# lmcinnes/pynndescent

Measured on AMD Instinct MI355X. Metric: index build: points indexed/sec (recall@10 vs brute force reported alongside), higher is better.
Workload: dtype f32

## Files before the change

pynndescent_amd/csrc/leaf_join.hip:

```cpp
#include <type_traits>

#include "common.h"
#include "metric.h"
#include "gram.h"
#include "merge.h"
#include "state.h"

#ifndef NND_LEAF_QW_OCC
#define NND_LEAF_QW_OCC 6
#endif
template <int NT, int NW, int DC, bool QW = false>
struct leaf_cfg {
    static constexpr int MP = NT * 16;
    static constexpr int TR = (NT + NW - 1) / NW;
    static constexpr int DSTRIDE = MP + 1;
    static constexpr int XS_FLOATS = MP * DC;
    static constexpr bool FULLD = NT <= 6;
    static constexpr int TPW = (NT * (NT + 1) / 2 + NW - 1) / NW;
    static constexpr int DB_FLOATS = FULLD ? MP * DSTRIDE : NW * 16 * DSTRIDE;
    static constexpr int QPASS = (MP + NW * 4 - 1) / (NW * 4);
    static constexpr bool PREFETCH = FULLD && !QW;
    static constexpr int PRE_FLOATS = PREFETCH ? MP * 16 * 2 : 0;
    static constexpr int EPI_FLOATS = DB_FLOATS + PRE_FLOATS;
    static constexpr int BIG_FLOATS = XS_FLOATS > EPI_FLOATS ? XS_FLOATS : EPI_FLOATS;
};

template <int NT, int NW, int DC, bool QW = false>
__global__ __launch_bounds__(NW * 64, (NT <= 5 && NW == 8) ? 8 : (QW && NT <= 5 && NW == 4) ? NND_LEAF_QW_OCC : 1) void k_leaf_join(const float *__restrict__ xp, int dp, const float *__restrict__ nrm,
                                                       int metric, const int32_t *__restrict__ perm,
                                                       const int32_t *__restrict__ wl_start,
                                                       const int32_t *__restrict__ wl_len, int64_t leaf0,
                                                       int64_t n_leaves, int k, int ks, uint32_t *__restrict__ knn_e,
                                                       float *__restrict__ knn_d, float *__restrict__ th,
                                                       long long *__restrict__ counters, int m_lo) {
    using C = leaf_cfg<NT, NW, DC, QW>;
    static_assert(!QW || C::FULLD, "quarter-wave merges read the whole distance block from LDS");
    __shared__ __attribute__((aligned(16))) float big[C::BIG_FLOATS];
    __shared__ int32_t ids[C::MP];
    __shared__ float nrs[C::MP];
    __shared__ uint2 qscr[QW ? NW * 4 * NND_Q16B_CAP : 1];
#ifdef NND_LEAF_PAD_LDS
    __shared__ float lds_pad[NND_LEAF_PAD_LDS];
    if (dp < 0) lds_pad[threadIdx.x] = 1.0f, counters[0] = (long long)lds_pad[(threadIdx.x + 1) & 63];
#endif

    const int tid = threadIdx.x, lane = nnd_lane(), w = tid >> 6;
    const int64_t leaf = leaf0 + blockIdx.x;
    if (leaf >= n_leaves) return;
    const int start = wl_start[leaf];
    const int m = wl_len[leaf];
    if (m < 2) return;
    if (m <= m_lo || m > C::MP) return;
    const int nt = (m + 15) >> 4;
    const int mp = nt << 4;

    for (int r = tid; r < C::MP; r += NW * 64) ids[r] = r < m ? perm[start + r] : -1;
    __syncthreads();

    constexpr int NTHR = NW * 64;
    constexpr int NLD = (C::MP * (DC / 4) + NTHR - 1) / NTHR;
    constexpr int NKL = (C::MP * 16 + NTHR - 1) / NTHR;
    constexpr bool quarter = QW;
    const bool use_pre = !quarter && C::PREFETCH && ks <= 16 && (m * ks * 2 <= C::BIG_FLOATS - C::DB_FLOATS);
    uint32_t qe[C::QPASS];
    float qd[C::QPASS];
    float *Xs = big;
    uint32_t pe[NKL];
    float pd[NKL];
    f32x4 acc[C::TR][NT];
    f32x4 acct[C::TPW];
    int tI[C::TPW], tJ[C::TPW];
    bool tOn[C::TPW];
#pragma unroll
    for (int tr = 0; tr < C::TR; tr++)
#pragma unroll
        for (int J = 0; J < NT; J++) acc[tr][J] = f32x4{0.f, 0.f, 0.f, 0.f};
#pragma unroll
    for (int q = 0; q < C::TPW; q++) {
        acct[q] = f32x4{0.f, 0.f, 0.f, 0.f};
        int t = w + q * NW, I = 0;
        while (I < nt && t >= nt - I) {
            t -= nt - I;
            I++;
        }
        tOn[q] = I < nt;
        tI[q] = I < nt ? I : 0;
        tJ[q] = I < nt ? I + t : 0;
    }

    for (int c0 = 0; c0 < dp; c0 += DC) {
        const int cw = (dp - c0) < DC ? (dp - c0) : DC;
        {
            static_assert(DC == 64, "cw is 32 or 64 (dp is a multiple of 32): chunk index by shift");
            const int nch = cw >> 2, total = mp * nch, nsh = cw == 64 ? 4 : 3;
            f32x4 rv[NLD];
#pragma unroll
            for (int q = 0; q < NLD; q++) {
                const int idx = tid + q * NTHR, idc = idx < total ? idx : 0;
                const int r = idc >> nsh, ch = idc & (nch - 1);
                const int id = ids[r];
                rv[q] = *(const f32x4 *)(xp + (int64_t)(id >= 0 ? id : 0) * dp + c0 + 4 * ch);
            }
            float my_nrm = 0.0f;
            if (c0 == 0) {
                if (!QW && tid < C::MP) {
                    const int id = ids[tid];
                    my_nrm = nrm[id >= 0 ? id : 0];
                }
                if constexpr (quarter) {
#pragma unroll
                    for (int q = 0; q < C::QPASS; q++) {
                        const int i = q * NW * 4 + (tid >> 4), j = lane & 15;
                        const bool on = i < m && j < k;
                        const int64_t v = ids[i < m ? i : 0];
                        const uint32_t ev = knn_e[v * ks + (on ? j : 0)];
                        const float dv = knn_d[v * ks + (on ? j : 0)];
                        qe[q] = on ? ev : NND_EMPTY_E;
                        qd[q] = on ? dv : INFINITY;
                    }
                }
                if (use_pre) {
#pragma unroll
                    for (int q = 0; q < NKL; q++) {
                        const int idx = tid + q * NTHR, idc = idx < m * ks ? idx : 0;
                        const int i = idc / ks, j = idc - i * ks;
                        pe[q] = knn_e[(int64_t)ids[i] * ks + j];
                        pd[q] = knn_d[(int64_t)ids[i] * ks + j];
                    }
                }
            }
            if (c0 > 0) __syncthreads();
#pragma unroll
            for (int q = 0; q < NLD; q++) {
                const int idx = tid + q * NTHR;
                if (idx < total) {
                    const int r = idx >> nsh, ch = idx & (nch - 1);
                    *(f32x4 *)&Xs[nnd_swz<DC>(r, ch)] = rv[q];
                }
            }
            if (!QW && c0 == 0 && tid < C::MP) nrs[tid] = my_nrm;
        }
        __syncthreads();
        if constexpr (C::FULLD) {
            const int lr = lane & 15, lg = lane >> 4;
            auto run = [&](auto nq_tag) {
                constexpr int NQ = decltype(nq_tag)::value;
#ifdef NND_LEAF_NOGRAM
                for (int t = 0; t < 1; t++) {
#else
                for (int t = 0; t < (cw >> 4); t++) {
#endif
                    const int c = 4 * t + lg;
                    float4 a[NQ], b[NQ];
#pragma unroll
                    for (int q = 0; q < NQ; q++) {
                        a[q] = *(const float4 *)&Xs[nnd_swz<DC>(tI[q] * 16 + lr, c)];
                        b[q] = *(const float4 *)&Xs[nnd_swz<DC>(tJ[q] * 16 + lr, c)];
                    }
#pragma unroll
                    for (int q = 0; q < NQ; q++) acct[q] = __builtin_amdgcn_mfma_f32_16x16x4f32(a[q].x, b[q].x, acct[q], 0, 0, 0);
#pragma unroll
                    for (int q = 0; q < NQ; q++) acct[q] = __builtin_amdgcn_mfma_f32_16x16x4f32(a[q].y, b[q].y, acct[q], 0, 0, 0);
#pragma unroll
                    for (int q = 0; q < NQ; q++) acct[q] = __builtin_amdgcn_mfma_f32_16x16x4f32(a[q].z, b[q].z, acct[q], 0, 0, 0);
#pragma unroll
                    for (int q = 0; q < NQ; q++) acct[q] = __builtin_amdgcn_mfma_f32_16x16x4f32(a[q].w, b[q].w, acct[q], 0, 0, 0);
                }
            };
            int nq = 0;
#pragma unroll
            for (int q = 0; q < C::TPW; q++) nq += tOn[q] ? 1 : 0;
            static_assert(C::TPW <= 4, "slot dispatch below");
            if (nq == 1) run(std::integral_constant<int, 1>{});
            else if (nq == 2) run(std::integral_constant<int, C::TPW >= 2 ? 2 : 1>{});
            else if (nq == 3) run(std::integral_constant<int, C::TPW >= 3 ? 3 : 1>{});
            else if (nq == 4) run(std::integral_constant<int, C::TPW >= 4 ? 4 : 1>{});
        } else {
#pragma unroll
            for (int tr = 0; tr < C::TR; tr++) {
                const int I = w + tr * NW;
                if (I < nt) nnd_gram_chunk<DC, NT>(Xs, I * 16, 0, cw, acc[tr], [nt](int J) { return J < nt; });
            }
        }
    }
    if constexpr (QW) {
        const int r16d = lane & 15, gd = lane >> 4;
#pragma unroll
        for (int q = 0; q < C::TPW; q++) {
            if (!tOn[q] || tI[q] != tJ[q]) continue;
#pragma unroll
            for (int r = 0; r < 4; r++)
                if (4 * gd + r == r16d) nrs[tI[q] * 16 + r16d] = acct[q][r];
        }
    }
    __syncthreads();

    const int r16 = lane & 15, g = lane >> 4;
    int accepted = 0;
    if constexpr (C::FULLD) {
        float *Dm = big;
#pragma unroll
        for (int q = 0; q < C::TPW; q++) {
            if (!tOn[q]) continue;
            const int I = tI[q], J = tJ[q];
            const int j = J * 16 + r16;
            const float nj = nrs[j];
#pragma unroll
            for (int r = 0; r < 4; r++) {
                const int il = I * 16 + 4 * g + r;
                const float dv = nnd_gram_to_dist<NND_CODES_ANY>(metric, acct[q][r], nrs[il], nj);
                Dm[il * C::DSTRIDE + j] = dv;
                if (I != J) Dm[j * C::DSTRIDE + il] = dv;
            }
        }
        uint32_t *pre_e = (uint32_t *)(big + C::DB_FLOATS);
        float *pre_d = big + C::DB_FLOATS + m * ks;
        if (use_pre) {
#pragma unroll
            for (int q = 0; q < NKL; q++) {
                const int idx = tid + q * NTHR;
                if (idx < m * ks) {
                    pre_e[idx] = pe[q];
                    pre_d[idx] = pd[q];
                }
            }
        }
        __syncthreads();
        if constexpr (quarter) {
#pragma unroll
            for (int q = 0; q < C::QPASS; q++) {
                if (q * NW * 4 + w * 4 >= m) break;
                const int i = q * NW * 4 + (tid >> 4);
                const bool on = i < m;
                const float *Drow = Dm + (on ? i : 0) * C::DSTRIDE;
                const int64_t v = ids[on ? i : 0];
#ifdef NND_LEAF_NOMERGE
                if (qe[q] == 12345u && qd[q] == 3.0f && Drow[lane] == 7.0f) accepted++;
                if (false)
#endif
#ifdef NND_LEAF_OLD_MERGE
                accepted += nnd_merge_rows_q16<NT>(on, knn_e + v * ks, knn_d + v * ks, th + v, qe[q], qd[q], k, m,
                                                   [&](int c, uint32_t &id, float &dc) {
                                                       id = (uint32_t)ids[c];
                                                       dc = Drow[c];
                                                       return c != i;
                                                   });
#else
                accepted += nnd_merge_rows_q16b<NT>(on, knn_e + v * ks, knn_d + v * ks, th + v, qe[q], qd[q], k, m,
                                                    [&](int c, uint32_t &id, float &dc) {
                                                        id = (uint32_t)ids[c];
                                                        dc = Drow[c];
                                                        return c != i;
                                                    }, qscr + w * 4 * NND_Q16B_CAP);
#endif
            }
        } else
        for (int i = w; i < m; i += NW) {
            const float *Drow = Dm + i * C::DSTRIDE;
            const int64_t v = ids[i];
            uint32_t e0 = NND_EMPTY_E;
            float d0 = INFINITY;
            if (lane < k) {
                if (use_pre) {
                    e0 = pre_e[i * ks + lane];
                    d0 = pre_d[i * ks + lane];
                } else {
                    e0 = knn_e[v * ks + lane];
                    d0 = knn_d[v * ks + lane];
                }
            }
            auto cf = [&](int c, uint32_t &id, float &dc) {
                id = (uint32_t)ids[c];
                dc = Drow[c];
                return c != i;
            };
#ifdef NND_LEAF_NOMERGE
            if (e0 == 12345u && d0 == 3.0f && Drow[lane] == 7.0f) accepted++;
            if (false)
#endif
            if (C::MP > 64 && m <= 64)
                accepted += nnd_merge_row_regs<1>(knn_e + v * ks, knn_d + v * ks, th + v, e0, d0, k, m, cf);
            else
                accepted += nnd_merge_row_regs<(C::MP + 63) / 64>(knn_e + v * ks, knn_d + v * ks, th + v, e0, d0, k, m, cf);
        }
    } else {
        float *Dw = big + w * 16 * C::DSTRIDE;
#pragma unroll
        for (int tr = 0; tr < C::TR; tr++) {
            const int I = w + tr * NW;
            if (I >= nt) continue;
#pragma unroll
            for (int J = 0; J < NT; J++) {
                if (J < nt) {
                    const int j = J * 16 + r16;
                    const float nj = nrs[j];
#pragma unroll
                    for (int r = 0; r < 4; r++) {
                        const int il = 4 * g + r;
                        Dw[il * C::DSTRIDE + j] = nnd_gram_to_dist<NND_CODES_ANY>(metric, acc[tr][J][r], nrs[I * 16 + il], nj);
                    }
                }
            }
            nnd_wave_lds_sync();
            const int lk = lane < k ? lane : 0;
            uint32_t e_nx = knn_e[(int64_t)ids[I * 16] * ks + lk];
            float d_nx = knn_d[(int64_t)ids[I * 16] * ks + lk];
            for (int il = 0; il < 16; il++) {
                const int i = I * 16 + il;
                if (i >= m) break;
                const float *Drow = Dw + il * C::DSTRIDE;
                const int64_t v = ids[i];
                const uint32_t e0 = lane < k ? e_nx : NND_EMPTY_E;
                const float d0 = lane < k ? d_nx : INFINITY;
                if (il + 1 < 16 && i + 1 < m) {
                    const int64_t vn = ids[i + 1];
                    e_nx = knn_e[vn * ks + lk];
                    d_nx = knn_d[vn * ks + lk];
                }
                accepted += nnd_merge_row_regs<(C::MP + 63) / 64>(knn_e + v * ks, knn_d + v * ks, th + v, e0, d0, k, m,
                                                                 [&](int c, uint32_t &id, float &dc) {
                                                                     id = (uint32_t)ids[c];
                                                                     dc = Drow[c];
                                                                     return c != i;
                                                                 });
            }
            nnd_wave_lds_sync();
        }
    }
    __syncthreads();
    int *wacc = (int *)nrs;
    if (lane == 0) wacc[w] = accepted;
    __syncthreads();
    if (tid == 0) {
        long long a = 0;
        for (int i = 0; i < NW; i++) a += wacc[i];
        nnd_count(counters, CNT_ACCEPT, a);
        nnd_count(counters, CNT_PAIRS, (long long)m * (m - 1) / 2);
        nnd_count(counters, CNT_ROWS, m);
        nnd_count(counters, CNT_MFMA, (long long)(C::FULLD ? nt * (nt + 1) / 2 : nt * nt) * (dp >> 2));
    }
}

template <int NT, int NW = 8, bool WIDE = false>
__global__ __launch_bounds__(NW * 64, 2) void k_leaf_join_rb(const float *__restrict__ xp, int dp, const float *__restrict__ nrm, int metric,
                                                         const int32_t *__restrict__ perm, const int32_t *__restrict__ wl_start,
                                                         const int32_t *__restrict__ wl_len, int64_t leaf0, int64_t n_leaves, int k, int ks,
                                                         uint32_t *__restrict__ knn_e, float *__restrict__ knn_d, float *__restrict__ th,
                                                         long long *__restrict__ counters) {
    constexpr int DC = 64, MP = NT * 16, RB = NW * 8, TRB = RB / 16, DSTRIDE = MP + 1;
    constexpr int TPW = (TRB * NT + NW - 1) / NW;
    constexpr int NLD = (MP * (DC / 4) + NW * 64 - 1) / (NW * 64);
    constexpr int BIG = MP * DC > RB * DSTRIDE ? MP * DC : RB * DSTRIDE;
    __shared__ __attribute__((aligned(16))) float big[BIG];
    __shared__ int32_t ids[MP];
    __shared__ float nrs[MP];
    __shared__ uint64_t wide_scr[WIDE ? NW : 1][WIDE ? NND_WIDE_SCRATCH_WORDS : 1];
    const int tid = threadIdx.x, lane = nnd_lane(), w = tid >> 6;
    const int64_t leaf = leaf0 + blockIdx.x;
    if (leaf >= n_leaves) return;
    const int start = wl_start[leaf], m = wl_len[leaf];
    const int r0 = blockIdx.y * RB;
    if (m < 2 || r0 >= m) return;
    const int nt = (m + 15) >> 4, mp = nt << 4;
    for (int r = tid; r < MP; r += NW * 64) {
        const int id = r < m ? perm[start + r] : -1;
        ids[r] = id;
        nrs[r] = nrm[id >= 0 ? id : 0];
    }
    __syncthreads();
    f32x4 acc[TPW];
    int tI[TPW], tJ[TPW];
    bool tOn[TPW];
#pragma unroll
    for (int q = 0; q < TPW; q++) {
        acc[q] = f32x4{0.f, 0.f, 0.f, 0.f};
        const int t = w + q * NW;
        const int I = t / nt, J = t - I * nt;
        tOn[q] = t < TRB * nt && (r0 >> 4) + I < nt;
        tI[q] = tOn[q] ? (r0 >> 4) + I : 0;
        tJ[q] = tOn[q] ? J : 0;
    }
    float *Xs = big;
    const int r16 = lane & 15, g = lane >> 4;
    for (int c0 = 0; c0 < dp; c0 += DC) {
        const int cw = (dp - c0) < DC ? (dp - c0) : DC;
        const int nch = cw >> 2, total = mp * nch, nsh = cw == 64 ? 4 : 3;
        f32x4 rv[NLD];
#pragma unroll
        for (int q = 0; q < NLD; q++) {
            const int idx = tid + q * NW * 64, idc = idx < total ? idx : 0;
            const int r = idc >> nsh, ch = idc & (nch - 1);
            const int id = ids[r];
            rv[q] = *(const f32x4 *)(xp + (int64_t)(id >= 0 ? id : 0) * dp + c0 + 4 * ch);
        }
        if (c0 > 0) __syncthreads();
#pragma unroll
        for (int q = 0; q < NLD; q++) {
            const int idx = tid + q * NW * 64;
            if (idx < total) {
                const int r = idx >> nsh, ch = idx & (nch - 1);
                *(f32x4 *)&Xs[nnd_swz<DC>(r, ch)] = rv[q];
            }
        }
        __syncthreads();
        for (int t = 0; t < (cw >> 4); t++) {
            const int c = 4 * t + g;
            float4 a[TPW], b[TPW];
#pragma unroll
            for (int q = 0; q < TPW; q++) {
                a[q] = *(const float4 *)&Xs[nnd_swz<DC>(tI[q] * 16 + r16, c)];
                b[q] = *(const float4 *)&Xs[nnd_swz<DC>(tJ[q] * 16 + r16, c)];
            }
#pragma unroll
            for (int q = 0; q < TPW; q++) acc[q] = __builtin_amdgcn_mfma_f32_16x16x4f32(a[q].x, b[q].x, acc[q], 0, 0, 0);
#pragma unroll
            for (int q = 0; q < TPW; q++) acc[q] = __builtin_amdgcn_mfma_f32_16x16x4f32(a[q].y, b[q].y, acc[q], 0, 0, 0);
#pragma unroll
            for (int q = 0; q < TPW; q++) acc[q] = __builtin_amdgcn_mfma_f32_16x16x4f32(a[q].z, b[q].z, acc[q], 0, 0, 0);
#pragma unroll
            for (int q = 0; q < TPW; q++) acc[q] = __builtin_amdgcn_mfma_f32_16x16x4f32(a[q].w, b[q].w, acc[q], 0, 0, 0);
        }
    }
// ... 163 lines not shown
        for (int r = 0; r < 4; r++) acc[q][r] = nnd_gram_to_dist<NND_CODES_ANY>(metric, acc[q][r], nrs[tI[q] * 16 + 4 * g + r], nj);
    }
    float *Dm = big;
    int accepted = 0;
    const int j32 = lane & 31, h = lane >> 5;
    for (int p0 = 0; p0 < m; p0 += RB) {
        uint32_t pe[SPW];
        float pd[SPW];
#pragma unroll
        for (int st = 0; st < SPW; st++) {
            const int i = p0 + w * (2 * SPW) + 2 * st + h;
            const bool on = i < m && j32 < k;
            const int64_t v = ids[i < m ? i : 0];
            const uint32_t ev = knn_e[v * ks + (on ? j32 : 0)];
            const float dv = knn_d[v * ks + (on ? j32 : 0)];
            pe[st] = on ? ev : NND_EMPTY_E;
            pd[st] = on ? dv : INFINITY;
        }
        __syncthreads();
#pragma unroll
        for (int q = 0; q < TPW; q++) {
            if (!tOn[q]) continue;
            const int I = tI[q], J = tJ[q];
            if (I * 16 >= p0 && I * 16 < p0 + RB) {
#pragma unroll
                for (int r = 0; r < 4; r++) Dm[(I * 16 + 4 * g + r - p0) * DSTRIDE + J * 16 + r16] = acc[q][r];
            }
            if (I != J && J * 16 >= p0 && J * 16 < p0 + RB) {
#pragma unroll
                for (int r = 0; r < 4; r++) Dm[(J * 16 + r16 - p0) * DSTRIDE + I * 16 + 4 * g + r] = acc[q][r];
            }
        }
        __syncthreads();
#pragma unroll
        for (int st = 0; st < SPW; st++) {
            if (p0 + w * (2 * SPW) + 2 * st >= m) break;
            const int i = p0 + w * (2 * SPW) + 2 * st + h;
            const bool on = i < m;
            const float *Drow = Dm + (on ? i - p0 : 0) * DSTRIDE;
            const int64_t v = ids[on ? i : 0];
            accepted += nnd_merge_rows_q32b(on, knn_e + v * ks, knn_d + v * ks, th + v, pe[st], pd[st], k, m,
                                            [&](int c, uint32_t &id, float &dc) {
                                                id = (uint32_t)ids[c];
                                                dc = Drow[c];
                                                return c != i;
                                            }, qscr + w * 2 * NND_Q32B_CAP);
        }
    }
    __syncthreads();
    int *wacc = (int *)nrs;
    if (lane == 0) wacc[w] = accepted;
    __syncthreads();
    if (tid == 0) {
        long long a = 0;
        for (int q = 0; q < NW; q++) a += wacc[q];
        nnd_count(counters, CNT_ACCEPT, a);
        nnd_count(counters, CNT_PAIRS, (long long)m * (m - 1) / 2);
        nnd_count(counters, CNT_ROWS, m);
        nnd_count(counters, CNT_MFMA, (long long)(nt * (nt + 1) / 2) * (dp >> 2));
    }
}

static constexpr int LEAF_MAX = 256;

static int run_leaf_rounds(nnd_ctx *ctx, const int32_t *perm, const int32_t *d_ws, const int32_t *d_wl,
                           const std::vector<int64_t> &tb, int maxlen) {
    if (nnd_zero_counters(ctx)) return 1;
    const int T = (int)tb.size() - 1;
    for (int t = 0; t < T; t++) {
        int64_t cnt = tb[t + 1] - tb[t];
        if (cnt <= 0) continue;
        dim3 grid((unsigned)cnt);
#define LEAF_ARGS ctx->xp, ctx->dp, ctx->nrm, ctx->p.metric, perm, d_ws, d_wl, tb[t], tb[t + 1], ctx->k, ctx->ks, \
                  ctx->knn_e, ctx->knn_d, ctx->th, ctx->counters
        const bool qw = ctx->k <= 16;
        if (ctx->k > NND_MAX_K) {
            if (maxlen <= 128)
                hipLaunchKernelGGL((k_leaf_join_rb<8, 8, true>), dim3((unsigned)cnt, 2), dim3(512), 0, ctx->stream, LEAF_ARGS);
            else if (maxlen <= 160)
                hipLaunchKernelGGL((k_leaf_join_rb<10, 8, true>), dim3((unsigned)cnt, 3), dim3(512), 0, ctx->stream, LEAF_ARGS);
            else
                hipLaunchKernelGGL((k_leaf_join_rb<16, 8, true>), dim3((unsigned)cnt, 4), dim3(512), 0, ctx->stream, LEAF_ARGS);
        }
#ifndef NND_LEAF_OLD_K32
        else if (!qw && ctx->k <= 32 && maxlen <= 160) {
            hipLaunchKernelGGL((k_leaf_join_sym<6, 8>), grid, dim3(512), 0, ctx->stream, LEAF_ARGS, 0);
            if (maxlen > 96) hipLaunchKernelGGL((k_leaf_join_sym<10, 8>), grid, dim3(512), 0, ctx->stream, LEAF_ARGS, 96);
        }
#endif
        else if (maxlen <= 64 && qw)
            hipLaunchKernelGGL((k_leaf_join<4, 8, 64, true>), grid, dim3(512), 0, ctx->stream, LEAF_ARGS, 0);
        else if (maxlen <= 64)
            hipLaunchKernelGGL((k_leaf_join<4, 8, 64>), grid, dim3(512), 0, ctx->stream, LEAF_ARGS, 0);
        else if (maxlen <= 80 && qw) {
#ifdef NND_LEAF_ONE_CLASS
            hipLaunchKernelGGL((k_leaf_join<5, 8, 64, true>), grid, dim3(512), 0, ctx->stream, LEAF_ARGS, 0);
#else
            hipLaunchKernelGGL((k_leaf_join<4, 4, 64, true>), grid, dim3(256), 0, ctx->stream, LEAF_ARGS, 0);
#ifdef NND_LEAF_EMPTY_L
            hipLaunchKernelGGL((k_leaf_join<5, 8, 64, true>), grid, dim3(512), 0, ctx->stream, LEAF_ARGS, 1000);
#elif defined(NND_LEAF_L_NW4)
            hipLaunchKernelGGL((k_leaf_join<5, 4, 64, true>), grid, dim3(256), 0, ctx->stream, LEAF_ARGS, 64);
#else
            hipLaunchKernelGGL((k_leaf_join<5, 8, 64, true>), grid, dim3(512), 0, ctx->stream, LEAF_ARGS, 64);
#endif
#endif
        }
        else if (maxlen <= 80)
            hipLaunchKernelGGL((k_leaf_join<5, 8, 64>), grid, dim3(512), 0, ctx->stream, LEAF_ARGS, 0);
        else if (maxlen <= 96 && qw)
            hipLaunchKernelGGL((k_leaf_join<6, 8, 64, true>), grid, dim3(512), 0, ctx->stream, LEAF_ARGS, 0);
        else if (maxlen <= 96)
            hipLaunchKernelGGL((k_leaf_join<6, 8, 64>), grid, dim3(512), 0, ctx->stream, LEAF_ARGS, 0);
        else if (maxlen <= 128)
            hipLaunchKernelGGL((k_leaf_join_rb<8, 8>), dim3((unsigned)cnt, 2), dim3(512), 0, ctx->stream, LEAF_ARGS);
        else if (maxlen <= 160)
            hipLaunchKernelGGL((k_leaf_join_rb<10, 8>), dim3((unsigned)cnt, 3), dim3(512), 0, ctx->stream, LEAF_ARGS);
        else
            hipLaunchKernelGGL((k_leaf_join_rb<16, 8>), dim3((unsigned)cnt, 4), dim3(512), 0, ctx->stream, LEAF_ARGS);
#undef LEAF_ARGS
    }
    NND_HIP_CHECK(hipGetLastError());
    if (nnd_read_counters(ctx)) return 1;
    ctx->stats.leaf_pairs = ctx->h_counters[CNT_PAIRS];
    ctx->stats.leaf_rows = ctx->h_counters[CNT_ROWS];
    ctx->stats.leaf_mfma = ctx->h_counters[CNT_MFMA];
    return 0;
}

int nnd_launch_leaf_init(nnd_ctx *ctx) {
    if (!ctx->forest_built || ctx->n_leaves == 0) return 0;
    const int T = (int)ctx->tree_leaf_begin.size() - 1;
    const int32_t *d_ws = ctx->leaf_start, *d_wl = ctx->leaf_len;
    std::vector<int64_t> tb(ctx->tree_leaf_begin.begin(), ctx->tree_leaf_begin.end());
    int maxlen = ctx->max_leaf;
    if (ctx->max_leaf > LEAF_MAX) {
        if (nnd_fetch_leaf_tables(ctx)) return 1;
        const std::vector<int32_t> &hs = ctx->h_leaf_start, &hl = ctx->h_leaf_len;
        std::vector<int32_t> ws, wl;
        ws.reserve(ctx->n_leaves);
        wl.reserve(ctx->n_leaves);
        maxlen = 0;
        for (int t = 0; t < T; t++) {
            tb[t] = (int64_t)ws.size();
            for (int64_t i = ctx->tree_leaf_begin[t]; i < ctx->tree_leaf_begin[t + 1]; i++) {
                int32_t a = hs[i], len = hl[i];
                while (len > 0) {
                    int32_t piece = len > LEAF_MAX ? LEAF_MAX : len;
                    ws.push_back(a);
                    wl.push_back(piece);
                    if (piece > maxlen) maxlen = piece;
                    a += piece;
                    len -= piece;
                }
            }
        }
        tb[T] = (int64_t)ws.size();
        const int64_t nw = (int64_t)ws.size();
        if (nw == 0) return 0;
        if (!ctx->mem.grow2(&ctx->wl_start, &ctx->wl_len, &ctx->wl_cap, nw, nw + nw / 4)) { ctx->set_error("out of device memory for the leaf work list"); return 1; }
        NND_HIP_CHECK(hipMemcpyAsync(ctx->wl_start, ws.data(), sizeof(int32_t) * nw, hipMemcpyHostToDevice, ctx->stream));
        NND_HIP_CHECK(hipMemcpyAsync(ctx->wl_len, wl.data(), sizeof(int32_t) * nw, hipMemcpyHostToDevice, ctx->stream));
        NND_HIP_CHECK(hipStreamSynchronize(ctx->stream));
        d_ws = ctx->wl_start;
        d_wl = ctx->wl_len;
    }
    return run_leaf_rounds(ctx, ctx->perm[ctx->cur], d_ws, d_wl, tb, maxlen);
}


int nnd_launch_leaf_init_array(nnd_ctx *ctx, const int32_t *leaf_host, int64_t n_leaves, int32_t max_leaf_size) {
    if (n_leaves <= 0 || max_leaf_size <= 0) return 0;
    const int64_t n = ctx->n;
    std::vector<int32_t> seen((size_t)n, 0);
    struct piece { int64_t off; int32_t len; int32_t round; };
    std::vector<piece> pieces;
    pieces.reserve((size_t)n_leaves);
    int n_rounds = 0, maxlen = 0;
    for (int64_t l = 0; l < n_leaves; l++) {
        const int32_t *row = leaf_host + l * max_leaf_size;
        int32_t len = 0;
        while (len < max_leaf_size && row[len] >= 0) {
            if ((int64_t)row[len] >= n) { ctx->set_error("nnd_init_from_leaf_array: leaf %lld holds point %d but n = %lld", (long long)l, row[len], (long long)n); return 1; }
            len++;
        }
        if (len < 2) continue;
        int32_t r = 0;
        for (int32_t i = 0; i < len; i++) r = seen[row[i]] > r ? seen[row[i]] : r;
        for (int32_t i = 0; i < len; i++) {
// ... 39 lines not shown
```

pynndescent_amd/csrc/merge.h:

```cpp
#pragma once
#include "common.h"

#define NND_MAX_K 64

__device__ __forceinline__ uint64_t nnd_readlane_u64(uint64_t v, int src_lane) {
    uint32_t lo = (uint32_t)__builtin_amdgcn_readlane((int)(uint32_t)v, src_lane);
    uint32_t hi = (uint32_t)__builtin_amdgcn_readlane((int)(uint32_t)(v >> 32), src_lane);
    return ((uint64_t)hi << 32) | lo;
}

template <int NCHUNK, typename CandFn>
__device__ __forceinline__ int nnd_merge_row_regs(uint32_t *__restrict__ row_e, float *__restrict__ row_d,
                                                  float *__restrict__ th_slot, uint32_t e, float d, int k, int ncand,
                                                  CandFn cand) {
    const int lane = nnd_lane();
    const uint64_t mykey = (e == NND_EMPTY_E) ? NND_EMPTY_KEY : nnd_make_key(d, e);
    const uint32_t myidx = e & NND_IDX_MASK;
    const float th = __int_as_float(__builtin_amdgcn_readlane(__float_as_int(d), k - 1));
    const int nlist = __popcll(__ballot(e != NND_EMPTY_E));

    uint32_t cid[NCHUNK];
    float cd[NCHUNK];
    unsigned long long cmask[NCHUNK];
    int nv = 0;
// ... 177 lines not shown
            u &= u - 1;
            if (u) {
                pnext = __builtin_ctz(u);
                nlo = (uint32_t)__builtin_amdgcn_ds_bpermute((gbase + pnext) << 2, (int)clo);
                nhi = (uint32_t)__builtin_amdgcn_ds_bpermute((gbase + pnext) << 2, (int)chi);
            }
            const uint64_t mykey = ((uint64_t)khi << 32) | klo, ck = ((uint64_t)bhi << 32) | blo;
            const bool gt = mykey > ck;
            const int gtl = nnd_dpp_row_shr1(gt ? 1 : 0);
            const uint32_t llo = (uint32_t)nnd_dpp_row_shr1((int)klo), lhi = (uint32_t)nnd_dpp_row_shr1((int)khi);
            const uint32_t lfl = (uint32_t)nnd_dpp_row_shr1((int)flag);
            if (gt) {
                klo = gtl ? llo : blo;
                khi = gtl ? lhi : bhi;
                flag = gtl ? lfl : NND_NEW_BIT;
            }
        }
    }
    if (pushed == 0) return 0;
    const bool empty = (klo & khi) == 0xFFFFFFFFu;
    e = empty ? NND_EMPTY_E : (klo | flag);
    d = empty ? INFINITY : __uint_as_float(khi);
    return pushed;
}

template <int NBLK, typename CandFn>
__device__ __forceinline__ int nnd_merge_rows_q16(bool row_on, uint32_t *__restrict__ row_e, float *__restrict__ row_d,
                                                  float *__restrict__ th_slot, uint32_t e, float d, int k, int ncand,
                                                  CandFn cand) {
    const int j = nnd_lane() & 15;
    const uint32_t e_in = e;
    const float d_in = d;
    const int pushed = nnd_merge_rows_q16_regs<NBLK>(row_on, e, d, k, ncand, cand);
    if (pushed == 0) return 0;
    if (row_on && j < k && (e != e_in || d != d_in)) {
        row_e[j] = e;
        row_d[j] = d;
        if (j == k - 1) *th_slot = d;
    }
    return pushed;
}

#define NND_Q16B_CAP 32
#define NND_DPP_QUAD_XOR1 0xB1
#define NND_DPP_QUAD_XOR2 0x4E
#define NND_DPP_QUAD_MIRROR 0x1B
#define NND_DPP_ROW_MIRROR 0x140
#define NND_DPP_ROW_HALF_MIRROR 0x141
#define NND_DPP_ROW_SHL(n) (0x100 + (n))

template <int CTRL>
__device__ __forceinline__ uint32_t nnd_q16_partner(uint32_t v) {
    if constexpr (CTRL >= 0) {
        return (uint32_t)__builtin_amdgcn_update_dpp(0, (int)v, CTRL, 0xF, 0xF, true);
    } else {
        const int t = __builtin_amdgcn_update_dpp(0, (int)v, NND_DPP_QUAD_MIRROR, 0xF, 0xF, true);
        return (uint32_t)__builtin_amdgcn_update_dpp(0, t, NND_DPP_ROW_HALF_MIRROR, 0xF, 0xF, true);
    }
}
template <int CTRL>
__device__ __forceinline__ void nnd_q16_cx(uint32_t &lo, uint32_t &hi, bool keep_max) {
    const uint32_t plo = nnd_q16_partner<CTRL>(lo), phi = nnd_q16_partner<CTRL>(hi);
    const bool less = (((uint64_t)phi << 32) | plo) < (((uint64_t)hi << 32) | lo);
    const bool take = less != keep_max;
    lo = take ? plo : lo;
    hi = take ? phi : hi;
}
template <int CTRL>
__device__ __forceinline__ void nnd_q16_cx(uint32_t &lo, uint32_t &hi, uint32_t &fl, bool keep_max) {
    const uint32_t plo = nnd_q16_partner<CTRL>(lo), phi = nnd_q16_partner<CTRL>(hi), pfl = nnd_q16_partner<CTRL>(fl);
    const bool less = (((uint64_t)phi << 32) | plo) < (((uint64_t)hi << 32) | lo);
    const bool take = less != keep_max;
    lo = take ? plo : lo;
    hi = take ? phi : hi;
    fl = take ? pfl : fl;
}
template <int T>
__device__ __forceinline__ bool nnd_q16_any_eq(uint32_t ids, uint32_t x) {
    if constexpr (T == 0) return ids == x;
    else return ((uint32_t)__builtin_amdgcn_update_dpp(0, (int)ids, NND_DPP_ROW_ROR(T), 0xF, 0xF, true) == x) | nnd_q16_any_eq<T - 1>(ids, x);
}

template <int NBLK, typename CandFn>
__device__ __forceinline__ int nnd_merge_rows_q16b(bool row_on, uint32_t *__restrict__ row_e, float *__restrict__ row_d,
                                                   float *__restrict__ th_slot, uint32_t e, float d, int k, int ncand,
                                                   CandFn cand, uint2 *wave_scr) {
    const int lane = nnd_lane(), j = lane & 15, gbase = lane & 48;
    uint2 *my = wave_scr + (lane >> 4) * NND_Q16B_CAP;
    const uint32_t e_in = e;
    const float d_in = d;
    uint32_t klo = e & NND_IDX_MASK, khi = __float_as_uint(d), flag = e & NND_NEW_BIT;
    if (e == NND_EMPTY_E) { klo = 0xFFFFFFFFu; khi = 0xFFFFFFFFu; flag = 0u; }
    const bool any_list = __ballot(e != NND_EMPTY_E) != 0;
    float th_cur = __int_as_float(__builtin_amdgcn_ds_bpermute((gbase + k - 1) << 2, __float_as_int(d)));
    const bool b0 = (j & 1) != 0, b1 = (j & 2) != 0, b2 = (j & 4) != 0, b3 = (j & 8) != 0;
    int fill = 0, pushed = 0;

    const int nblk = (ncand + 15) >> 4;
#pragma unroll 1
    for (int blk = 0; blk < nblk; blk++) {
        const int c = blk * 16 + j;
        uint32_t cid = 0;
        float dc = 0.0f;
        bool ok = row_on && c < ncand && cand(c, cid, dc);
        ok = ok && (dc < th_cur);
        const unsigned long long cmask = __ballot(ok);
        if (cmask) {
            const uint32_t m16 = (uint32_t)(cmask >> gbase) & 0xFFFFu;
            if (ok) my[fill + __popc(m16 & ((1u << j) - 1u))] = make_uint2(cid, __float_as_uint(dc));
            fill += __popc(m16);
        }
        const bool last = blk + 1 >= nblk;
        if (!__ballot(fill > 16 || (fill > 0 && (last || th_cur == INFINITY)))) continue;
        nnd_wave_lds_sync();
#pragma unroll 1
        for (int b = 0; b < NND_Q16B_CAP / 16; b++) {
            if (!__ballot(fill > 16 * b)) break;
            const uint2 s = my[16 * b + j];
            bool sok = 16 * b + j < fill && __uint_as_float(s.y) < th_cur;
            if (any_list && __ballot(sok)) {
                const bool dup = nnd_q16_any_eq<15>(klo, s.x);
                sok = sok && !dup;
            }
            const unsigned long long mask = __ballot(sok);
            if (!mask) continue;
            pushed += __popcll(mask);
            uint32_t slo = sok ? s.x : 0xFFFFFFFFu, shi = sok ? s.y : 0xFFFFFFFFu;
            nnd_q16_cx<NND_DPP_QUAD_XOR1>(slo, shi, b0);
            nnd_q16_cx<NND_DPP_QUAD_MIRROR>(slo, shi, b1);
            nnd_q16_cx<NND_DPP_QUAD_XOR1>(slo, shi, b0);
            nnd_q16_cx<NND_DPP_ROW_HALF_MIRROR>(slo, shi, b2);
            nnd_q16_cx<NND_DPP_QUAD_XOR2>(slo, shi, b1);
            nnd_q16_cx<NND_DPP_QUAD_XOR1>(slo, shi, b0);
            nnd_q16_cx<NND_DPP_ROW_MIRROR>(slo, shi, b3);
            nnd_q16_cx<-1>(slo, shi, b2);
            nnd_q16_cx<NND_DPP_QUAD_XOR2>(slo, shi, b1);
            nnd_q16_cx<NND_DPP_QUAD_XOR1>(slo, shi, b0);
            {
                const uint32_t tlo = nnd_q16_partner<NND_DPP_ROW_MIRROR>(slo), thi = nnd_q16_partner<NND_DPP_ROW_MIRROR>(shi);
                const bool take = (((uint64_t)thi << 32) | tlo) < (((uint64_t)khi << 32) | klo);
                klo = take ? tlo : klo;
                khi = take ? thi : khi;
                flag = take ? NND_NEW_BIT : flag;
            }
            nnd_q16_cx<NND_DPP_ROW_ROR(8)>(klo, khi, flag, b3);
            nnd_q16_cx<-1>(klo, khi, flag, b2);
            nnd_q16_cx<NND_DPP_QUAD_XOR2>(klo, khi, flag, b1);
            nnd_q16_cx<NND_DPP_QUAD_XOR1>(klo, khi, flag, b0);
            if (j >= k) { klo = 0xFFFFFFFFu; khi = 0xFFFFFFFFu; flag = 0u; }
            const uint32_t wk = (uint32_t)__builtin_amdgcn_ds_bpermute((gbase + k - 1) << 2, (int)khi);
            th_cur = wk == 0xFFFFFFFFu ? INFINITY : __uint_as_float(wk);
        }
        fill = 0;
        nnd_wave_lds_sync();
    }
    if (pushed == 0) return 0;
    const bool empty = (klo & khi) == 0xFFFFFFFFu;
    e = empty ? NND_EMPTY_E : (klo | flag);
    d = empty ? INFINITY : __uint_as_float(khi);
    if (row_on && j < k && (e != e_in || d != d_in)) {
        row_e[j] = e;
        row_d[j] = d;
        if (j == k - 1) *th_slot = d;
    }
    return pushed;
}

#define NND_Q32B_CAP 64
template <int PX>
__device__ __forceinline__ uint32_t nnd_q32_partner(uint32_t v, int lane) {
    if constexpr (PX == 1) return nnd_q16_partner<NND_DPP_QUAD_XOR1>(v);
    else if constexpr (PX == 2) return nnd_q16_partner<NND_DPP_QUAD_XOR2>(v);
    else if constexpr (PX == 3) return nnd_q16_partner<NND_DPP_QUAD_MIRROR>(v);
    else if constexpr (PX == 4) return nnd_q16_partner<-1>(v);
    else if constexpr (PX == 7) return nnd_q16_partner<NND_DPP_ROW_HALF_MIRROR>(v);
    else if constexpr (PX == 8) return nnd_q16_partner<NND_DPP_ROW_ROR(8)>(v);
    else if constexpr (PX == 15) return nnd_q16_partner<NND_DPP_ROW_MIRROR>(v);
    else return (uint32_t)__builtin_amdgcn_ds_bpermute((lane ^ PX) << 2, (int)v);
}
template <int PX>
__device__ __forceinline__ void nnd_q32_cx(uint32_t &lo, uint32_t &hi, bool keep_max, int lane) {
    const uint32_t plo = nnd_q32_partner<PX>(lo, lane), phi = nnd_q32_partner<PX>(hi, lane);
    const bool take = ((((uint64_t)phi << 32) | plo) < (((uint64_t)hi << 32) | lo)) != keep_max;
    lo = take ? plo : lo;
    hi = take ? phi : hi;
}
template <int PX>
__device__ __forceinline__ void nnd_q32_cx(uint32_t &lo, uint32_t &hi, uint32_t &fl, bool keep_max, int lane) {
    const uint32_t plo = nnd_q32_partner<PX>(lo, lane), phi = nnd_q32_partner<PX>(hi, lane), pfl = nnd_q32_partner<PX>(fl, lane);
    const bool take = ((((uint64_t)phi << 32) | plo) < (((uint64_t)hi << 32) | lo)) != keep_max;
    lo = take ? plo : lo;
    hi = take ? phi : hi;
    fl = take ? pfl : fl;
}

template <typename CandFn>
__device__ __forceinline__ int nnd_merge_rows_q32b(bool row_on, uint32_t *__restrict__ row_e, float *__restrict__ row_d,
                                                   float *__restrict__ th_slot, uint32_t e, float d, int k, int ncand,
                                                   CandFn cand, uint2 *wave_scr) {
    const int lane = nnd_lane(), j = lane & 31, gb = lane & 32;
    uint2 *my = wave_scr + (lane >> 5) * NND_Q32B_CAP;
    const uint32_t e_in = e;
    const float d_in = d;
    uint32_t klo = e & NND_IDX_MASK, khi = __float_as_uint(d), flag = e & NND_NEW_BIT;
    if (e == NND_EMPTY_E) { klo = 0xFFFFFFFFu; khi = 0xFFFFFFFFu; flag = 0u; }
    const bool any_list = __ballot(e != NND_EMPTY_E) != 0;
    float th_cur = __int_as_float(__builtin_amdgcn_ds_bpermute((gb + k - 1) << 2, __float_as_int(d)));
    const bool b0 = (j & 1) != 0, b1 = (j & 2) != 0, b2 = (j & 4) != 0, b3 = (j & 8) != 0, b4 = (j & 16) != 0;
    const uint32_t below = (1u << j) - 1u;
    int fill = 0, pushed = 0;
    const int nblk = (ncand + 31) >> 5;
#pragma unroll 1
    for (int blk = 0; blk < nblk; blk++) {
        const int c = blk * 32 + j;
        uint32_t cid = 0;
        float dc = 0.0f;
        bool ok = row_on && c < ncand && cand(c, cid, dc);
        ok = ok && (dc < th_cur);
        const unsigned long long cmask = __ballot(ok);
        if (cmask) {
            const uint32_t m32 = (uint32_t)(cmask >> gb);
            if (ok) my[fill + __popc(m32 & below)] = make_uint2(cid, __float_as_uint(dc));
            fill += __popc(m32);
        }
        const bool last = blk + 1 >= nblk;
        if (!__ballot(fill > 32 || (fill > 0 && (last || th_cur == INFINITY)))) continue;
        nnd_wave_lds_sync();
#pragma unroll 1
        for (int b = 0; b < NND_Q32B_CAP / 32; b++) {
            if (!__ballot(fill > 32 * b)) break;
            const uint2 s = my[32 * b + j];
            bool sok = 32 * b + j < fill && __uint_as_float(s.y) < th_cur;
            if (any_list && __ballot(sok)) {
                const uint32_t other = (uint32_t)__builtin_amdgcn_ds_bpermute((lane ^ 16) << 2, (int)klo);
                const bool dup0 = nnd_q16_any_eq<15>(klo, s.x), dup1 = nnd_q16_any_eq<15>(other, s.x);
                const bool dup = dup0 || dup1;
                sok = sok && !dup;
            }
            const unsigned long long mask = __ballot(sok);
            if (!mask) continue;
            pushed += __popcll(mask);
            uint32_t slo = sok ? s.x : 0xFFFFFFFFu, shi = sok ? s.y : 0xFFFFFFFFu;
            nnd_q32_cx<1>(slo, shi, b0, lane);
            nnd_q32_cx<3>(slo, shi, b1, lane);
            nnd_q32_cx<1>(slo, shi, b0, lane);
            nnd_q32_cx<7>(slo, shi, b2, lane);
            nnd_q32_cx<2>(slo, shi, b1, lane);
            nnd_q32_cx<1>(slo, shi, b0, lane);
// ... 127 lines not shown
```

Baseline: 54.51 million.

## Prune dead leaf-join paths, precompute swizzled Gram addresses, shorten partial bitonic sorts

```diff
diff --git a/pynndescent_amd/csrc/leaf_join.hip b/pynndescent_amd/csrc/leaf_join.hip
--- a/pynndescent_amd/csrc/leaf_join.hip
+++ b/pynndescent_amd/csrc/leaf_join.hip
@@ -12,17 +12,13 @@
 template <int NT, int NW, int DC, bool QW = false>
 struct leaf_cfg {
     static constexpr int MP = NT * 16;
-    static constexpr int TR = (NT + NW - 1) / NW;
     static constexpr int DSTRIDE = MP + 1;
     static constexpr int XS_FLOATS = MP * DC;
-    static constexpr bool FULLD = NT <= 6;
+    static_assert(NT <= 6, "the distance block of the whole leaf in LDS");
     static constexpr int TPW = (NT * (NT + 1) / 2 + NW - 1) / NW;
-    static constexpr int DB_FLOATS = FULLD ? MP * DSTRIDE : NW * 16 * DSTRIDE;
+    static constexpr int DB_FLOATS = MP * DSTRIDE;
     static constexpr int QPASS = (MP + NW * 4 - 1) / (NW * 4);
-    static constexpr bool PREFETCH = FULLD && !QW;
-    static constexpr int PRE_FLOATS = PREFETCH ? MP * 16 * 2 : 0;
-    static constexpr int EPI_FLOATS = DB_FLOATS + PRE_FLOATS;
-    static constexpr int BIG_FLOATS = XS_FLOATS > EPI_FLOATS ? XS_FLOATS : EPI_FLOATS;
+    static constexpr int BIG_FLOATS = XS_FLOATS > DB_FLOATS ? XS_FLOATS : DB_FLOATS;
 };
 
 template <int NT, int NW, int DC, bool QW = false>
@@ -34,15 +30,10 @@
                                                        float *__restrict__ knn_d, float *__restrict__ th,
                                                        long long *__restrict__ counters, int m_lo) {
     using C = leaf_cfg<NT, NW, DC, QW>;
-    static_assert(!QW || C::FULLD, "quarter-wave merges read the whole distance block from LDS");
     __shared__ __attribute__((aligned(16))) float big[C::BIG_FLOATS];
     __shared__ int32_t ids[C::MP];
     __shared__ float nrs[C::MP];
     __shared__ uint2 qscr[QW ? NW * 4 * NND_Q16B_CAP : 1];
-#ifdef NND_LEAF_PAD_LDS
-    __shared__ float lds_pad[NND_LEAF_PAD_LDS];
-    if (dp < 0) lds_pad[threadIdx.x] = 1.0f, counters[0] = (long long)lds_pad[(threadIdx.x + 1) & 63];
-#endif
 
     const int tid = threadIdx.x, lane = nnd_lane(), w = tid >> 6;
     const int64_t leaf = leaf0 + blockIdx.x;
@@ -59,22 +50,13 @@
 
     constexpr int NTHR = NW * 64;
     constexpr int NLD = (C::MP * (DC / 4) + NTHR - 1) / NTHR;
-    constexpr int NKL = (C::MP * 16 + NTHR - 1) / NTHR;
     constexpr bool quarter = QW;
-    const bool use_pre = !quarter && C::PREFETCH && ks <= 16 && (m * ks * 2 <= C::BIG_FLOATS - C::DB_FLOATS);
     uint32_t qe[C::QPASS];
     float qd[C::QPASS];
     float *Xs = big;
-    uint32_t pe[NKL];
-    float pd[NKL];
-    f32x4 acc[C::TR][NT];
     f32x4 acct[C::TPW];
     int tI[C::TPW], tJ[C::TPW];
     bool tOn[C::TPW];
-#pragma unroll
-    for (int tr = 0; tr < C::TR; tr++)
-#pragma unroll
-        for (int J = 0; J < NT; J++) acc[tr][J] = f32x4{0.f, 0.f, 0.f, 0.f};
 #pragma unroll
     for (int q = 0; q < C::TPW; q++) {
         acct[q] = f32x4{0.f, 0.f, 0.f, 0.f};
@@ -119,15 +101,6 @@
                         qd[q] = on ? dv : INFINITY;
                     }
                 }
-                if (use_pre) {
-#pragma unroll
-                    for (int q = 0; q < NKL; q++) {
-                        const int idx = tid + q * NTHR, idc = idx < m * ks ? idx : 0;
-                        const int i = idc / ks, j = idc - i * ks;
-                        pe[q] = knn_e[(int64_t)ids[i] * ks + j];
-                        pd[q] = knn_d[(int64_t)ids[i] * ks + j];
-                    }
-                }
             }
             if (c0 > 0) __syncthreads();
 #pragma unroll
@@ -141,21 +114,18 @@
             if (!QW && c0 == 0 && tid < C::MP) nrs[tid] = my_nrm;
         }
         __syncthreads();
-        if constexpr (C::FULLD) {
+        {
             const int lr = lane & 15, lg = lane >> 4;
             auto run = [&](auto nq_tag) {
                 constexpr int NQ = decltype(nq_tag)::value;
-#ifdef NND_LEAF_NOGRAM
-                for (int t = 0; t < 1; t++) {
-#else
+                const int lane_b = (lr * DC + ((lg ^ (lr & 3)) << 2)) * 4, x_b = (lr >> 2) << 6;
                 for (int t = 0; t < (cw >> 4); t++) {
-#endif
-                    const int c = 4 * t + lg;
+                    const int t_b = ((t << 6) ^ x_b) + lane_b;
                     float4 a[NQ], b[NQ];
 #pragma unroll
                     for (int q = 0; q < NQ; q++) {
-                        a[q] = *(const float4 *)&Xs[nnd_swz<DC>(tI[q] * 16 + lr, c)];
-                        b[q] = *(const float4 *)&Xs[nnd_swz<DC>(tJ[q] * 16 + lr, c)];
+                        a[q] = *(const float4 *)((const char *)Xs + (t_b + tI[q] * (16 * DC * 4)));
+                        b[q] = *(const float4 *)((const char *)Xs + (t_b + tJ[q] * (16 * DC * 4)));
                     }
 #pragma unroll
                     for (int q = 0; q < NQ; q++) acct[q] = __builtin_amdgcn_mfma_f32_16x16x4f32(a[q].x, b[q].x, acct[q], 0, 0, 0);
@@ -175,12 +145,6 @@
             else if (nq == 2) run(std::integral_constant<int, C::TPW >= 2 ? 2 : 1>{});
             else if (nq == 3) run(std::integral_constant<int, C::TPW >= 3 ? 3 : 1>{});
             else if (nq == 4) run(std::integral_constant<int, C::TPW >= 4 ? 4 : 1>{});
-        } else {
-#pragma unroll
-            for (int tr = 0; tr < C::TR; tr++) {
-                const int I = w + tr * NW;
-                if (I < nt) nnd_gram_chunk<DC, NT>(Xs, I * 16, 0, cw, acc[tr], [nt](int J) { return J < nt; });
-            }
         }
     }
     if constexpr (QW) {
@@ -197,7 +161,7 @@
 
     const int r16 = lane & 15, g = lane >> 4;
     int accepted = 0;
-    if constexpr (C::FULLD) {
+    {
         float *Dm = big;
 #pragma unroll
         for (int q = 0; q < C::TPW; q++) {
@@ -211,18 +175,6 @@
                 const float dv = nnd_gram_to_dist<NND_CODES_ANY>(metric, acct[q][r], nrs[il], nj);
                 Dm[il * C::DSTRIDE + j] = dv;
                 if (I != J) Dm[j * C::DSTRIDE + il] = dv;
-            }
-        }
-        uint32_t *pre_e = (uint32_t *)(big + C::DB_FLOATS);
-        float *pre_d = big + C::DB_FLOATS + m * ks;
-        if (use_pre) {
-#pragma unroll
-            for (int q = 0; q < NKL; q++) {
-                const int idx = tid + q * NTHR;
-                if (idx < m * ks) {
-                    pre_e[idx] = pe[q];
-                    pre_d[idx] = pd[q];
-                }
             }
         }
         __syncthreads();
@@ -234,25 +186,12 @@
                 const bool on = i < m;
                 const float *Drow = Dm + (on ? i : 0) * C::DSTRIDE;
                 const int64_t v = ids[on ? i : 0];
-#ifdef NND_LEAF_NOMERGE
-                if (qe[q] == 12345u && qd[q] == 3.0f && Drow[lane] == 7.0f) accepted++;
-                if (false)
-#endif
-#ifdef NND_LEAF_OLD_MERGE
-                accepted += nnd_merge_rows_q16<NT>(on, knn_e + v * ks, knn_d + v * ks, th + v, qe[q], qd[q], k, m,
-                                                   [&](int c, uint32_t &id, float &dc) {
-                                                       id = (uint32_t)ids[c];
-                                                       dc = Drow[c];
-                                                       return c != i;
-                                                   });
-#else
-                accepted += nnd_merge_rows_q16b<NT>(on, knn_e + v * ks, knn_d + v * ks, th + v, qe[q], qd[q], k, m,
-                                                    [&](int c, uint32_t &id, float &dc) {
-                                                        id = (uint32_t)ids[c];
-                                                        dc = Drow[c];
-                                                        return c != i;
-                                                    }, qscr + w * 4 * NND_Q16B_CAP);
-#endif
+                nnd_merge_rows_q16b<NT>(on, knn_e + v * ks, knn_d + v * ks, th + v, qe[q], qd[q], k, m,
+                                        [&](int c, uint32_t &id, float &dc) {
+                                            id = (uint32_t)ids[c];
+                                            dc = Drow[c];
+                                            return c != i;
+                                        }, qscr + w * 4 * NND_Q16B_CAP);
             }
         } else
         for (int i = w; i < m; i += NW) {
@@ -261,83 +200,35 @@
             uint32_t e0 = NND_EMPTY_E;
             float d0 = INFINITY;
             if (lane < k) {
-                if (use_pre) {
-                    e0 = pre_e[i * ks + lane];
-                    d0 = pre_d[i * ks + lane];
-                } else {
-                    e0 = knn_e[v * ks + lane];
-                    d0 = knn_d[v * ks + lane];
-                }
+                e0 = knn_e[v * ks + lane];
+                d0 = knn_d[v * ks + lane];
             }
             auto cf = [&](int c, uint32_t &id, float &dc) {
                 id = (uint32_t)ids[c];
                 dc = Drow[c];
                 return c != i;
             };
-#ifdef NND_LEAF_NOMERGE
-            if (e0 == 12345u && d0 == 3.0f && Drow[lane] == 7.0f) accepted++;
-            if (false)
-#endif
             if (C::MP > 64 && m <= 64)
                 accepted += nnd_merge_row_regs<1>(knn_e + v * ks, knn_d + v * ks, th + v, e0, d0, k, m, cf);
             else
                 accepted += nnd_merge_row_regs<(C::MP + 63) / 64>(knn_e + v * ks, knn_d + v * ks, th + v, e0, d0, k, m, cf);
         }
-    } else {
-        float *Dw = big + w * 16 * C::DSTRIDE;
-#pragma unroll
-        for (int tr = 0; tr < C::TR; tr++) {
-            const int I = w + tr * NW;
-            if (I >= nt) continue;
-#pragma unroll
-            for (int J = 0; J < NT; J++) {
-                if (J < nt) {
-                    const int j = J * 16 + r16;
-                    const float nj = nrs[j];
-#pragma unroll
-                    for (int r = 0; r < 4; r++) {
-                        const int il = 4 * g + r;
-                        Dw[il * C::DSTRIDE + j] = nnd_gram_to_dist<NND_CODES_ANY>(metric, acc[tr][J][r], nrs[I * 16 + il], nj);
-                    }
-                }
-            }
-            nnd_wave_lds_sync();
-            const int lk = lane < k ? lane : 0;
-            uint32_t e_nx = knn_e[(int64_t)ids[I * 16] * ks + lk];
-            float d_nx = knn_d[(int64_t)ids[I * 16] * ks + lk];
-            for (int il = 0; il < 16; il++) {
-                const int i = I * 16 + il;
-                if (i >= m) break;
-                const float *Drow = Dw + il * C::DSTRIDE;
-                const int64_t v = ids[i];
-                const uint32_t e0 = lane < k ? e_nx : NND_EMPTY_E;
-                const float d0 = lane < k ? d_nx : INFINITY;
-                if (il + 1 < 16 && i + 1 < m) {
-                    const int64_t vn = ids[i + 1];
-                    e_nx = knn_e[vn * ks + lk];
-                    d_nx = knn_d[vn * ks + lk];
-                }
-                accepted += nnd_merge_row_regs<(C::MP + 63) / 64>(knn_e + v * ks, knn_d + v * ks, th + v, e0, d0, k, m,
-                                                                 [&](int c, uint32_t &id, float &dc) {
-                                                                     id = (uint32_t)ids[c];
-                                                                     dc = Drow[c];
-                                                                     return c != i;
-                                                                 });
-            }
-            nnd_wave_lds_sync();
-        }
-    }
-    __syncthreads();
+    }
     int *wacc = (int *)nrs;
-    if (lane == 0) wacc[w] = accepted;
-    __syncthreads();
+    if constexpr (!QW) {
+        __syncthreads();
+        if (lane == 0) wacc[w] = accepted;
+        __syncthreads();
+    }
     if (tid == 0) {
-        long long a = 0;
-        for (int i = 0; i < NW; i++) a += wacc[i];
-        nnd_count(counters, CNT_ACCEPT, a);
+        if constexpr (!QW) {
+            long long a = 0;
+            for (int i = 0; i < NW; i++) a += wacc[i];
+            nnd_count(counters, CNT_ACCEPT, a);
+        }
         nnd_count(counters, CNT_PAIRS, (long long)m * (m - 1) / 2);
         nnd_count(counters, CNT_ROWS, m);
-        nnd_count(counters, CNT_MFMA, (long long)(C::FULLD ? nt * (nt + 1) / 2 : nt * nt) * (dp >> 2));
+        nnd_count(counters, CNT_MFMA, (long long)(nt * (nt + 1) / 2) * (dp >> 2));
     }
 }
 
@@ -667,29 +558,17 @@
             else
                 hipLaunchKernelGGL((k_leaf_join_rb<16, 8, true>), dim3((unsigned)cnt, 4), dim3(512), 0, ctx->stream, LEAF_ARGS);
         }
-#ifndef NND_LEAF_OLD_K32
         else if (!qw && ctx->k <= 32 && maxlen <= 160) {
             hipLaunchKernelGGL((k_leaf_join_sym<6, 8>), grid, dim3(512), 0, ctx->stream, LEAF_ARGS, 0);
             if (maxlen > 96) hipLaunchKernelGGL((k_leaf_join_sym<10, 8>), grid, dim3(512), 0, ctx->stream, LEAF_ARGS, 96);
         }
-#endif
         else if (maxlen <= 64 && qw)
             hipLaunchKernelGGL((k_leaf_join<4, 8, 64, true>), grid, dim3(512), 0, ctx->stream, LEAF_ARGS, 0);
         else if (maxlen <= 64)
             hipLaunchKernelGGL((k_leaf_join<4, 8, 64>), grid, dim3(512), 0, ctx->stream, LEAF_ARGS, 0);
         else if (maxlen <= 80 && qw) {
-#ifdef NND_LEAF_ONE_CLASS
-            hipLaunchKernelGGL((k_leaf_join<5, 8, 64, true>), grid, dim3(512), 0, ctx->stream, LEAF_ARGS, 0);
-#else
             hipLaunchKernelGGL((k_leaf_join<4, 4, 64, true>), grid, dim3(256), 0, ctx->stream, LEAF_ARGS, 0);
-#ifdef NND_LEAF_EMPTY_L
-            hipLaunchKernelGGL((k_leaf_join<5, 8, 64, true>), grid, dim3(512), 0, ctx->stream, LEAF_ARGS, 1000);
-#elif defined(NND_LEAF_L_NW4)
-            hipLaunchKernelGGL((k_leaf_join<5, 4, 64, true>), grid, dim3(256), 0, ctx->stream, LEAF_ARGS, 64);
-#else
             hipLaunchKernelGGL((k_leaf_join<5, 8, 64, true>), grid, dim3(512), 0, ctx->stream, LEAF_ARGS, 64);
-#endif
-#endif
         }
         else if (maxlen <= 80)
             hipLaunchKernelGGL((k_leaf_join<5, 8, 64>), grid, dim3(512), 0, ctx->stream, LEAF_ARGS, 0);
diff --git a/pynndescent_amd/csrc/merge.h b/pynndescent_amd/csrc/merge.h
--- a/pynndescent_amd/csrc/merge.h
+++ b/pynndescent_amd/csrc/merge.h
@@ -283,19 +283,20 @@
 }
 
 template <int NBLK, typename CandFn>
-__device__ __forceinline__ int nnd_merge_rows_q16b(bool row_on, uint32_t *__restrict__ row_e, float *__restrict__ row_d,
-                                                   float *__restrict__ th_slot, uint32_t e, float d, int k, int ncand,
-                                                   CandFn cand, uint2 *wave_scr) {
+__device__ __forceinline__ void nnd_merge_rows_q16b(bool row_on, uint32_t *__restrict__ row_e, float *__restrict__ row_d,
+                                                    float *__restrict__ th_slot, uint32_t e, float d, int k, int ncand,
+                                                    CandFn cand, uint2 *wave_scr) {
     const int lane = nnd_lane(), j = lane & 15, gbase = lane & 48;
     uint2 *my = wave_scr + (lane >> 4) * NND_Q16B_CAP;
     const uint32_t e_in = e;
     const float d_in = d;
     uint32_t klo = e & NND_IDX_MASK, khi = __float_as_uint(d), flag = e & NND_NEW_BIT;
     if (e == NND_EMPTY_E) { klo = 0xFFFFFFFFu; khi = 0xFFFFFFFFu; flag = 0u; }
-    const bool any_list = __ballot(e != NND_EMPTY_E) != 0;
+    bool any_list = __ballot(e != NND_EMPTY_E) != 0;
     float th_cur = __int_as_float(__builtin_amdgcn_ds_bpermute((gbase + k - 1) << 2, __float_as_int(d)));
     const bool b0 = (j & 1) != 0, b1 = (j & 2) != 0, b2 = (j & 4) != 0, b3 = (j & 8) != 0;
-    int fill = 0, pushed = 0;
+    int fill = 0;
+    bool folded = false;
 
     const int nblk = (ncand + 15) >> 4;
 #pragma unroll 1
@@ -318,36 +319,51 @@
         for (int b = 0; b < NND_Q16B_CAP / 16; b++) {
             if (!__ballot(fill > 16 * b)) break;
             const uint2 s = my[16 * b + j];
-            bool sok = 16 * b + j < fill && __uint_as_float(s.y) < th_cur;
+            const int cnt = fill - 16 * b;
+            bool sok = j < cnt && __uint_as_float(s.y) < th_cur;
             if (any_list && __ballot(sok)) {
                 const bool dup = nnd_q16_any_eq<15>(klo, s.x);
                 sok = sok && !dup;
             }
-            const unsigned long long mask = __ballot(sok);
-            if (!mask) continue;
-            pushed += __popcll(mask);
+            if (!__ballot(sok)) continue;
+            folded = true;
             uint32_t slo = sok ? s.x : 0xFFFFFFFFu, shi = sok ? s.y : 0xFFFFFFFFu;
-            nnd_q16_cx<NND_DPP_QUAD_XOR1>(slo, shi, b0);
-            nnd_q16_cx<NND_DPP_QUAD_MIRROR>(slo, shi, b1);
-            nnd_q16_cx<NND_DPP_QUAD_XOR1>(slo, shi, b0);
-            nnd_q16_cx<NND_DPP_ROW_HALF_MIRROR>(slo, shi, b2);
-            nnd_q16_cx<NND_DPP_QUAD_XOR2>(slo, shi, b1);
-            nnd_q16_cx<NND_DPP_QUAD_XOR1>(slo, shi, b0);
-            nnd_q16_cx<NND_DPP_ROW_MIRROR>(slo, shi, b3);
-            nnd_q16_cx<-1>(slo, shi, b2);
-            nnd_q16_cx<NND_DPP_QUAD_XOR2>(slo, shi, b1);
-            nnd_q16_cx<NND_DPP_QUAD_XOR1>(slo, shi, b0);
-            {
-                const uint32_t tlo = nnd_q16_partner<NND_DPP_ROW_MIRROR>(slo), thi = nnd_q16_partner<NND_DPP_ROW_MIRROR>(shi);
-                const bool take = (((uint64_t)thi << 32) | tlo) < (((uint64_t)khi << 32) | klo);
-                klo = take ? tlo : klo;
-                khi = take ? thi : khi;
-                flag = take ? NND_NEW_BIT : flag;
-            }
-            nnd_q16_cx<NND_DPP_ROW_ROR(8)>(klo, khi, flag, b3);
-            nnd_q16_cx<-1>(klo, khi, flag, b2);
-            nnd_q16_cx<NND_DPP_QUAD_XOR2>(klo, khi, flag, b1);
-            nnd_q16_cx<NND_DPP_QUAD_XOR1>(klo, khi, flag, b0);
+            if (__ballot(cnt > 1)) {
+                nnd_q16_cx<NND_DPP_QUAD_XOR1>(slo, shi, b0);
+                if (__ballot(cnt > 2)) {
+                    nnd_q16_cx<NND_DPP_QUAD_MIRROR>(slo, shi, b1);
+                    nnd_q16_cx<NND_DPP_QUAD_XOR1>(slo, shi, b0);
+                    if (__ballot(cnt > 4)) {
+                        nnd_q16_cx<NND_DPP_ROW_HALF_MIRROR>(slo, shi, b2);
+                        nnd_q16_cx<NND_DPP_QUAD_XOR2>(slo, shi, b1);
+                        nnd_q16_cx<NND_DPP_QUAD_XOR1>(slo, shi, b0);
+                        if (__ballot(cnt > 8)) {
+                            nnd_q16_cx<NND_DPP_ROW_MIRROR>(slo, shi, b3);
+                            nnd_q16_cx<-1>(slo, shi, b2);
+                            nnd_q16_cx<NND_DPP_QUAD_XOR2>(slo, shi, b1);
+                            nnd_q16_cx<NND_DPP_QUAD_XOR1>(slo, shi, b0);
+                        }
+                    }
+                }
+            }
+            if (!any_list) {
+                klo = slo;
+                khi = shi;
+                flag = (slo & shi) == 0xFFFFFFFFu ? 0u : NND_NEW_BIT;
+                any_list = true;
+            } else {
+                {
+                    const uint32_t tlo = nnd_q16_partner<NND_DPP_ROW_MIRROR>(slo), thi = nnd_q16_partner<NND_DPP_ROW_MIRROR>(shi);
+                    const bool take = (((uint64_t)thi << 32) | tlo) < (((uint64_t)khi << 32) | klo);
+                    klo = take ? tlo : klo;
+                    khi = take ? thi : khi;
+                    flag = take ? NND_NEW_BIT : flag;
+                }
+                nnd_q16_cx<NND_DPP_ROW_ROR(8)>(klo, khi, flag, b3);
+                nnd_q16_cx<-1>(klo, khi, flag, b2);
+                nnd_q16_cx<NND_DPP_QUAD_XOR2>(klo, khi, flag, b1);
+                nnd_q16_cx<NND_DPP_QUAD_XOR1>(klo, khi, flag, b0);
+            }
             if (j >= k) { klo = 0xFFFFFFFFu; khi = 0xFFFFFFFFu; flag = 0u; }
             const uint32_t wk = (uint32_t)__builtin_amdgcn_ds_bpermute((gbase + k - 1) << 2, (int)khi);
             th_cur = wk == 0xFFFFFFFFu ? INFINITY : __uint_as_float(wk);
@@ -355,7 +371,7 @@
         fill = 0;
         nnd_wave_lds_sync();
     }
-    if (pushed == 0) return 0;
+    if (!folded) return;
     const bool empty = (klo & khi) == 0xFFFFFFFFu;
     e = empty ? NND_EMPTY_E : (klo | flag);
     d = empty ? INFINITY : __uint_as_float(khi);
@@ -364,7 +380,6 @@
         row_d[j] = d;
         if (j == k - 1) *th_slot = d;
     }
-    return pushed;
 }
 
 #define NND_Q32B_CAP 64
```

After: 54.76 million (median of 4 runs). About the same (+0.5%).
